# fschmid56/EfficientAT

Hardware: NVIDIA H100
Metric: clips/sec (10s@32kHz) mn10_as fwd+bwd (higher is better)
Workload: dtype f32

## Files before the change

efficientat_b200/engine.py:

```python
import os

import torch

from ._lib import check_module_tensors, lib

ACT = {"none": 0, "relu": 1, "hswish": 2}
BN_EPS = 1e-3
BN_MOM = 0.01


def _ptr(t):
    return 0 if t is None else t.data_ptr()


def _stream():
    return torch.cuda.current_stream().cuda_stream


def _conv_out(n, k, s):
    return (n + 2 * ((k - 1) // 2) - k) // s + 1


class _Layer:
    pass


SE_FUSED_DEFAULT = "1"


DGRAD_BNRED_DEFAULT = "0"


DW_BWD_FUSED_DEFAULT = "1"
DW_BWD_FUSED_SHAPES = ((3, 1), (3, 2), (5, 2))


class _ZeroPool:

    def __init__(self, chunk=1 << 16):
        self.chunk, self.buf, self.off = chunk, None, 0

    def take(self, rows, cols, dev):
        n = rows * cols
        if self.buf is None or self.off + n > self.buf.numel() or self.buf.device != dev:
            self.buf = torch.zeros(max(self.chunk, n), device=dev, dtype=torch.float64)
            self.off = 0
        v = self.buf[self.off:self.off + n].view(rows, cols)
        self.off += n
        return v


class _Fork:

    def __init__(self, device, enabled):
        self.enabled = enabled
        self.side = torch.cuda.Stream(device) if enabled else None
        self.keep = []

    def run(self, fn, *tensors):
        if not self.enabled:
            fn()
            return
        self.side.wait_stream(torch.cuda.current_stream())
        with torch.cuda.stream(self.side):
            fn()
        self.keep.extend(tensors)

    def join(self):
        if self.enabled:
            torch.cuda.current_stream().wait_stream(self.side)
            self.keep.clear()


class MNEngine:
    def __init__(self, model):
        self.model = model
        self.precision = getattr(model, "precision", "fp32")
        if self.precision not in ("fp32", "bf16"):
            raise ValueError(f"precision must be 'fp32' or 'bf16', got {self.precision}")
        self.gemm_impl = os.environ.get("EAT_GEMM", "auto")
        self.tc_min_rows = 1024
        self.pw_impl = "tc" if os.environ.get("EAT_PW_IMPL") == "tc" else "tma"
        self.fork_wgrad = os.environ.get("EAT_FORK_WGRAD", "0") == "1"
        self.se_fused = os.environ.get("EAT_SE_FUSED", SE_FUSED_DEFAULT) == "1"
        self.se_parts_per_sm = int(os.environ.get("EAT_SE_PARTS_PER_SM", "6"))
        self.dgrad_bnred = os.environ.get("EAT_DGRAD_BNRED", DGRAD_BNRED_DEFAULT) == "1"
        self.dw_bwd_fused = os.environ.get("EAT_DW_BWD_FUSED", DW_BWD_FUSED_DEFAULT) == "1"
        self._fork = None
        self._se_scale = {}
        self._zero_pool = _ZeroPool()
        self._plan()

    def _plan(self):
        from .models.mn.block_types import ConcurrentSEBlock, ConvNormActivation, InvertedResidual
        feats = list(self.model.features)
        self.stem = feats[0]
        self.last = feats[-1]
        self.blocks = []
        for m in feats[1:-1]:
            assert isinstance(m, InvertedResidual)
            L = _Layer()
            subs = list(m.block)
            L.expand = L.se = None
            i = 0
            if len([s for s in subs if isinstance(s, ConvNormActivation)]) == 3:
                L.expand = subs[0]
                i = 1
            L.dw = subs[i]
            i += 1
            if isinstance(subs[i], ConcurrentSEBlock):
                L.se = subs[i].conc_se_layers[0]
                i += 1
            L.proj = subs[i]
            L.res = m.use_res_connect
            L.act = ACT["hswish"] if m.cnf.use_hs else ACT["relu"]
            L.k = m.cnf.kernel
            L.stride = m.cnf.stride
            L.cin, L.cexp, L.cout = m.cnf.input_channels, m.cnf.expanded_channels, m.cnf.out_channels
            self.blocks.append(L)
        self.fc1 = self.model.classifier[2]
        self.fc2 = self.model.classifier[5]
        self.dropout_p = self.model.classifier[4].p

    @property
    def tdtype(self):
        return torch.float32 if self.precision == "fp32" else torch.bfloat16

    @property
    def dcode(self):
        return 0 if self.precision == "fp32" else 1

    def _gemm(self, a, w, out, M, N, K, in_sc=None, in_act=0, gate=None, rows_per_sample=1, sc=None, bias=None,
              act=0, res=None, stats=None, a_code=None, c_code=None, w_trans=False):
        a_code = self.dcode if a_code is None else a_code
        c_code = self.dcode if c_code is None else c_code
        scale = _ptr(sc[0]) if sc is not None else 0
        shift = _ptr(sc[1]) if sc is not None else _ptr(bias)
        args = (a.data_ptr(), a_code, w.data_ptr(), 1 if w_trans else 0, out.data_ptr(), c_code, M, N, K,
                _ptr(in_sc[0]) if in_sc is not None else 0, _ptr(in_sc[1]) if in_sc is not None else 0, in_act,
                _ptr(gate), rows_per_sample, scale, shift, act, _ptr(res),
                _ptr(stats[0]) if stats is not None else 0, _ptr(stats[1]) if stats is not None else 0, _stream())
        L = lib()
        use_tc = (self.gemm_impl != "simt" and a_code == c_code and M >= self.tc_min_rows and K % 8 == 0
                  and N % 8 == 0 and act != 3 and in_act != 3)
        if use_tc and a_code == 0 and self.pw_impl == "tma" and not (res is not None and act != 0):
            ws = torch.empty(N * ((K + 31) // 32) * 128, device=w.device, dtype=torch.uint8)
            L.pw_tma_fwd(a.data_ptr(), w.data_ptr(), 1 if w_trans else 0, out.data_ptr(), M, N, K, args[9], args[10], in_act,
                         _ptr(gate), rows_per_sample, scale, shift, act, _ptr(res), args[18], args[19], ws.data_ptr(),
                         ws.numel(), _stream())
        elif use_tc:
            if w_trans:
                wt = torch.empty(N, K, device=w.device, dtype=torch.float32)
                L.transpose_f32(w.data_ptr(), wt.data_ptr(), K, N, _stream())
                args = (args[0], args[1], wt.data_ptr(), 0) + args[4:]
            L.pw_tc_fwd(*args)
        else:
            L.gemm_simt_fwd(*args)

    def _fold(self, bn, dev):
        c = bn.num_features
        sc = torch.empty(2, c, device=dev, dtype=torch.float32)
        lib().bn_fold(bn.weight.data_ptr(), bn.bias.data_ptr(), bn.running_mean.data_ptr(),
                      bn.running_var.data_ptr(), bn.eps, sc[0].data_ptr(), sc[1].data_ptr(), c, _stream())
        return sc

    def _finalize(self, bn, stats, count, dev):
        c = bn.num_features
        sc = torch.empty(2, c, device=dev, dtype=torch.float32)
        sv = torch.empty(2, c, device=dev, dtype=torch.float32)
        mom = bn.momentum if bn.momentum is not None else 0.1
        track = bn.track_running_stats and bn.running_mean is not None
        lib().bn_finalize(stats[0].data_ptr(), stats[1].data_ptr(), float(count), bn.weight.data_ptr(),
                          bn.bias.data_ptr(), bn.eps, mom, _ptr(bn.running_mean) if track else 0,
                          _ptr(bn.running_var) if track else 0, _ptr(bn.num_batches_tracked) if track else 0,
                          sc[0].data_ptr(), sc[1].data_ptr(), sv[0].data_ptr(), sv[1].data_ptr(), c, _stream())
        return sc, sv

    def _se_gate(self, se, pool, inv_count, B, C, dev, hidden=None):
        S = se.fc1.out_features
        key = (S, float(inv_count), str(dev))
        sc = self._se_scale.get(key)
        if sc is None:
            sc = torch.full((S,), float(inv_count), device=dev, dtype=torch.float32)
            self._se_scale[key] = sc
        if hidden is None:
            hidden = torch.empty(B, S, device=dev, dtype=torch.float32)
        self._gemm(pool, se.fc1.weight, hidden, B, S, C, sc=(sc, se.fc1.bias), act=ACT["relu"], a_code=0, c_code=0)
        gate = torch.empty(B, C, device=dev, dtype=torch.float32)
        self._gemm(hidden, se.fc2.weight, gate, B, C, S, bias=se.fc2.bias, act=3, a_code=0, c_code=0)
        return gate, hidden

    def _dw_weights(self, conv, dev):
        c, k = conv.out_channels, conv.kernel_size[0]
        wt = torch.empty(k * k, c, device=dev, dtype=torch.float32)
        lib().dw_repack(conv.weight.data_ptr(), wt.data_ptr(), c, k, _stream())
        return wt

    def forward(self, x, return_fmaps=False):
        if not x.is_cuda:
            raise RuntimeError("efficientat_b200 models run on CUDA (sm_90a) only; got a CPU tensor")
        if x.dim() != 4 or x.shape[1] != 1:
            raise ValueError(f"expected input of shape [B, 1, F, T], got {tuple(x.shape)}")
        check_module_tensors(self.model, x.device, type(self.model).__name__)
        self.dropout_p = float(self.model.classifier[4].p)
        needs_grad = torch.is_grad_enabled() and any(p.requires_grad for p in self.model.parameters())
        with torch.cuda.device(x.device):
            if self.model.training:
                if return_fmaps:
                    raise NotImplementedError("return_fmaps is available in eval mode only")
                from .autograd import mn_train_forward
                logits, feat = mn_train_forward(self, x, needs_grad)
                return self._squeeze(logits, feat) + (None,)
            if needs_grad and x.requires_grad:
                raise NotImplementedError("gradients w.r.t. the input spectrogram are not implemented")
            logits, feat, fmaps = self._forward_eval(x.detach(), return_fmaps)
            return self._squeeze(logits, feat) + (fmaps,)

    @staticmethod
    def _squeeze(logits, feat):
        return logits, feat

    def _forward_eval(self, x, return_fmaps=False):
        L = lib()
        dev = x.device
        st = _stream()
        td, dc = self.tdtype, self.dcode
        x = x.float().contiguous()
        B, _, F, T = x.shape
        fmaps = [] if return_fmaps else None

        def keep(t, f, tt, c):
            if fmaps is not None:
                fmaps.append(t.view(B, f, tt, c).permute(0, 3, 1, 2))

        conv, bn = self.stem[0], self.stem[1]
        s0 = conv.stride[0]
        Fi, Ti = _conv_out(F, 3, s0), _conv_out(T, 3, s0)
        c0 = conv.out_channels
        a = torch.empty(B, Fi, Ti, c0, device=dev, dtype=td)
        sc = self._fold(bn, dev)
# ... 151 lines not shown
                      Fi * Ti, cl, st)
        S["last"] = dict(inp=a, z=zl, sc=scl, sv=svl, Fi=Fi, Ti=Ti)
        n1 = self.fc1.out_features
        h_pre = torch.empty(B, n1, device=dev, dtype=torch.float32)
        self._gemm(feat, self.fc1.weight, h_pre, B, n1, cl, bias=self.fc1.bias, a_code=0, c_code=0)
        p = self.dropout_p
        if dropout_mask is None and p > 0:
            dropout_mask = torch.empty(B, n1, device=dev, dtype=torch.float32).bernoulli_(1.0 - p).div_(1.0 - p)
        ident = self._ident(n1, dev)
        logits = torch.empty(B, self.fc2.out_features, device=dev, dtype=torch.float32)
        self._gemm(h_pre, self.fc2.weight, logits, B, self.fc2.out_features, n1, in_sc=ident, in_act=HS,
                   gate=dropout_mask, rows_per_sample=1, bias=self.fc2.bias, a_code=0, c_code=0)
        S["head"] = dict(feat=feat, h_pre=h_pre, mask=dropout_mask, ident=ident)
        return logits, feat

    def _ident(self, n, dev):
        t = torch.empty(2, n, device=dev, dtype=torch.float32)
        t[0].fill_(1.0)
        t[1].zero_()
        return t

    def _block_modules(self):
        return list(self.model.features)[1:-1]

    def param_list(self):
        return [p for p in self.model.parameters()]

    def _wgrad(self, g, a, dW, db, M, N, K, in_sc=None, in_act=0, gate=None, rows_per_sample=1, g_code=None,
               a_code=None):
        g_code = self.dcode if g_code is None else g_code
        a_code = self.dcode if a_code is None else a_code
        args = (g.data_ptr(), g_code, a.data_ptr(), a_code, dW.data_ptr(), _ptr(db), M, N, K,
                _ptr(in_sc[0]) if in_sc is not None else 0, _ptr(in_sc[1]) if in_sc is not None else 0,
                in_act, _ptr(gate), rows_per_sample, _stream())
        use_tc = (self.gemm_impl != "simt" and db is None and g_code == a_code and M >= self.tc_min_rows
                  and K % 8 == 0 and N % 8 == 0)
        if use_tc:
            lib().pw_tc_wgrad(*args)
        else:
            lib().gemm_simt_wgrad(*args)

    def _bn_bwd_coef(self, gA, gate, dpool, z, sc, sv, act, B, P, C, dgamma, dbeta, dev, code, sums):
        L = lib()
        st = _stream()
        if sums is None:
            s = self._zero_pool.take(2, C, dev)
            L.bn_bwd_reduce(_ptr(gA), _ptr(gate), _ptr(dpool), z.data_ptr(), sc[0].data_ptr(), sc[1].data_ptr(),
                            sv[0].data_ptr(), sv[1].data_ptr(), act, code, B, P, C, s[0].data_ptr(), s[1].data_ptr(), st)
        else:
            s = sums
        coef = torch.empty(2, C, device=dev, dtype=torch.float32)
        L.bn_bwd_finalize(s[0].data_ptr(), s[1].data_ptr(), float(B * P), _ptr(dgamma), _ptr(dbeta),
                          coef[0].data_ptr(), coef[1].data_ptr(), C, st)
        return coef

    def _bn_bwd(self, gA, gate, dpool, z, sc, sv, act, B, P, C, dgamma, dbeta, dev, code=None, sums=None):
        L = lib()
        st = _stream()
        code = self.dcode if code is None else code
        coef = self._bn_bwd_coef(gA, gate, dpool, z, sc, sv, act, B, P, C, dgamma, dbeta, dev, code, sums)
        dz = torch.empty_like(z)
        L.bn_bwd_apply(_ptr(gA), _ptr(gate), _ptr(dpool), z.data_ptr(), sc[0].data_ptr(), sc[1].data_ptr(),
                       sv[0].data_ptr(), sv[1].data_ptr(), act, coef[0].data_ptr(), coef[1].data_ptr(), dz.data_ptr(),
                       code, B, P, C, st)
        return dz

    def _block_bwd(self, blk, R, dy, G, B):
        return self._ir_block_bwd(blk, R, dy, G, B)

    def _ir_block_bwd(self, blk, R, dy, G, B):
        L = lib()
        st = _stream()
        dev = dy.device
        td, dc = self.tdtype, self.dcode
        Fi, Ti, Fo, To = R["Fi"], R["Ti"], R["Fo"], R["To"]
        Pi, Po = Fi * Ti, Fo * To
        gate = R.get("gate")
        dz3 = self._bn_bwd(dy, None, None, R["z3"], R["sc3"], R["sv3"], 0, B, Po, blk.cout,
                           G[blk.proj[1].weight], G[blk.proj[1].bias], dev)
        fork = self._fork if self._fork is not None else _Fork(dev, False)
        fork.run(lambda: self._wgrad(dz3, R["z2"], G[blk.proj[0].weight], None, B * Po, blk.cout, blk.cexp, in_sc=R["sc2"],
                                     in_act=blk.act, gate=gate, rows_per_sample=Po), dz3)
        dp = torch.empty_like(R["z2"])
        self._gemm(dz3, blk.proj[0].weight, dp, B * Po, blk.cexp, blk.cout, w_trans=True)
        dpool = None
        if blk.se is not None:
            Sq = blk.se.fc1.out_features
            dgate = torch.zeros(B, blk.cexp, device=dev, dtype=torch.float32)
            if self.se_fused:
                parts = max(1, min(32, (torch.cuda.get_device_properties(dev).multi_processor_count * self.se_parts_per_sm) // B, (Po + 15) // 16))
                part = torch.empty(parts, 4, B, blk.cexp, device=dev, dtype=torch.float32)
                L.se_bn_bwd_reduce(dp.data_ptr(), R["z2"].data_ptr(), R["sc2"][0].data_ptr(), R["sc2"][1].data_ptr(),
                                   R["sv2"][0].data_ptr(), blk.act, dgate.data_ptr(), part.data_ptr(), parts, dc, B, Po,
                                   blk.cexp, st)
            else:
                L.se_bwd_reduce(dp.data_ptr(), R["z2"].data_ptr(), R["sc2"][0].data_ptr(), R["sc2"][1].data_ptr(),
                                blk.act, dgate.data_ptr(), dc, B, Po, blk.cexp, st)
            du2 = torch.empty(B, blk.cexp, device=dev, dtype=torch.float32)
            du1 = torch.empty(B, Sq, device=dev, dtype=torch.float32)
            dpool = torch.empty(B, blk.cexp, device=dev, dtype=torch.float32)
            L.se_fc_bwd(dgate.data_ptr(), gate.data_ptr(), R["hidden"].data_ptr(), blk.se.fc1.weight.data_ptr(),
                        blk.se.fc2.weight.data_ptr(), 1.0 / Po, du2.data_ptr(), du1.data_ptr(), dpool.data_ptr(),
                        B, blk.cexp, Sq, st)
            fork.run(lambda: (self._wgrad(du2, R["hidden"], G[blk.se.fc2.weight], G[blk.se.fc2.bias], B, blk.cexp, Sq, g_code=0, a_code=0),
                              self._wgrad(du1, R["mean"], G[blk.se.fc1.weight], G[blk.se.fc1.bias], B, Sq, blk.cexp, g_code=0, a_code=0)),
                     du2, du1)
        sums2 = None
        if blk.se is not None and self.se_fused:
            sums2 = self._zero_pool.take(2, blk.cexp, dev)
            L.se_bn_bwd_combine(part.data_ptr(), parts, gate.data_ptr(), dpool.data_ptr(), R["sv2"][1].data_ptr(), B,
                                blk.cexp, sums2[0].data_ptr(), sums2[1].data_ptr(), st)
        has_exp = blk.expand is not None
        dw_in = R["z1"] if has_exp else R["inp"]
        sc1 = R["sc1"] if has_exp else None
        if (self.dw_bwd_fused and dc == 0 and (blk.k, blk.stride) in DW_BWD_FUSED_SHAPES
                and blk.cexp % (4 if blk.k == 3 else 2) == 0):
            coef = self._bn_bwd_coef(dp, gate, dpool, R["z2"], R["sc2"], R["sv2"], blk.act, B, Po, blk.cexp,
                                     G[blk.dw[1].weight], G[blk.dw[1].bias], dev, dc, sums2)
            da1 = torch.empty_like(dw_in)
            sums1 = self._zero_pool.take(2, blk.cexp, dev) if has_exp else None
            L.dw_conv_bwd_fused(dp.data_ptr(), _ptr(gate), _ptr(dpool), R["z2"].data_ptr(), R["sc2"][0].data_ptr(),
                                R["sc2"][1].data_ptr(), R["sv2"][0].data_ptr(), R["sv2"][1].data_ptr(), blk.act,
                                coef[0].data_ptr(), coef[1].data_ptr(), R["wt"].data_ptr(), dw_in.data_ptr(),
                                _ptr(sc1[0]) if has_exp else 0, _ptr(sc1[1]) if has_exp else 0, blk.act if has_exp else 0,
                                _ptr(dy) if (blk.res and not has_exp) else 0, da1.data_ptr(),
                                G[blk.dw[0].weight].data_ptr(), _ptr(R["sv1"][0]) if has_exp else 0,
                                _ptr(R["sv1"][1]) if has_exp else 0, _ptr(sums1[0]) if has_exp else 0,
                                _ptr(sums1[1]) if has_exp else 0, dc, B, Fi, Ti, blk.cexp, blk.k, blk.stride, st)
            return self._expand_bwd(blk, R, dy, G, B, da1, sums1)
        dz2 = self._bn_bwd(dp, gate, dpool, R["z2"], R["sc2"], R["sv2"], blk.act, B, Po, blk.cexp,
                           G[blk.dw[1].weight], G[blk.dw[1].bias], dev, sums=sums2)
        fork.run(lambda: L.dw_conv_wgrad(dz2.data_ptr(), dw_in.data_ptr(), _ptr(sc1[0]) if has_exp else 0,
                                         _ptr(sc1[1]) if has_exp else 0, blk.act if has_exp else 0,
                                         G[blk.dw[0].weight].data_ptr(), 0, dc, B, Fi, Ti, blk.cexp, blk.k, blk.stride,
                                         _stream()), dz2)
        da1 = torch.empty_like(dw_in)
        sums1 = None
        if has_exp and self.dgrad_bnred and blk.stride == 2 and dc == 0 and blk.k in (3, 5):
            sums1 = self._zero_pool.take(2, blk.cexp, dev)
            L.dw_conv_dgrad_bnred(dz2.data_ptr(), R["wt"].data_ptr(), 0, da1.data_ptr(), R["z1"].data_ptr(),
                                  R["sc1"][0].data_ptr(), R["sc1"][1].data_ptr(), R["sv1"][0].data_ptr(),
                                  R["sv1"][1].data_ptr(), blk.act, sums1[0].data_ptr(), sums1[1].data_ptr(), dc, B, Fi, Ti,
                                  blk.cexp, blk.k, blk.stride, st)
        else:
            L.dw_conv_dgrad(dz2.data_ptr(), R["wt"].data_ptr(), 0, _ptr(dy) if (blk.res and not has_exp) else 0,
                            da1.data_ptr(), dc, B, Fi, Ti, blk.cexp, blk.k, blk.stride, st)
        return self._expand_bwd(blk, R, dy, G, B, da1, sums1)

    def _expand_bwd(self, blk, R, dy, G, B, da1, sums1):
        if blk.expand is None:
            return da1
        dev = da1.device
        Pi = R["Fi"] * R["Ti"]
        fork = self._fork if self._fork is not None else _Fork(dev, False)
        dz1 = self._bn_bwd(da1, None, None, R["z1"], R["sc1"], R["sv1"], blk.act, B, Pi, blk.cexp,
                           G[blk.expand[1].weight], G[blk.expand[1].bias], dev, sums=sums1)
        fork.run(lambda: self._wgrad(dz1, R["inp"], G[blk.expand[0].weight], None, B * Pi, blk.cexp, blk.cin), dz1)
        dinp = torch.empty_like(R["inp"])
        self._gemm(dz1, blk.expand[0].weight, dinp, B * Pi, blk.cin, blk.cexp, w_trans=True,
                   res=dy if blk.res else None)
        return dinp

    def _backward(self, S, dlogits, on_ready=None):
        L = lib()
        st = _stream()
        dev = dlogits.device
        td, dc = self.tdtype, self.dcode
        B = S["B"]
        HS = ACT["hswish"]
        self._zero_pool = _ZeroPool()
        params = self.param_list()
        flat = torch.zeros(sum(p.numel() for p in params), device=dev, dtype=torch.float32)
        G, off = {}, 0
        for p in params:
            G[p] = flat[off:off + p.numel()].view_as(p)
            off += p.numel()
        dlogits = dlogits.float().contiguous()
        fork = self._fork = _Fork(dev, self.fork_wgrad)
        pidx = {id(p): i for i, p in enumerate(params)}

        def done(module):
            fork.join()
            if on_ready is not None:
                on_ready(flat, min(pidx[id(p)] for p in module.parameters()))

        H = S["head"]
        n1, ncls, cl = self.fc1.out_features, self.fc2.out_features, self.fc1.in_features
        fork.run(lambda: self._wgrad(dlogits, H["h_pre"], G[self.fc2.weight], G[self.fc2.bias], B, ncls, n1, in_sc=H["ident"],
                                     in_act=HS, gate=H["mask"], rows_per_sample=1, g_code=0, a_code=0), dlogits)
        dh = torch.empty(B, n1, device=dev, dtype=torch.float32)
        self._gemm(dlogits, self.fc2.weight, dh, B, n1, ncls, a_code=0, c_code=0, w_trans=True)
        dpre = torch.empty_like(dh)
        L.act_bwd(dh.data_ptr(), H["h_pre"].data_ptr(), _ptr(H["mask"]), HS, dpre.data_ptr(), dh.numel(), st)
        fork.run(lambda: self._wgrad(dpre, H["feat"], G[self.fc1.weight], G[self.fc1.bias], B, n1, cl, g_code=0, a_code=0), dpre)
        dfeat = torch.empty(B, cl, device=dev, dtype=torch.float32)
        self._gemm(dpre, self.fc1.weight, dfeat, B, cl, n1, a_code=0, c_code=0, w_trans=True)
        done(self.fc1)

        Ls = S["last"]
        P = Ls["Fi"] * Ls["Ti"]
        conv, bn = self.last[0], self.last[1]
        dpool = dfeat.mul_(1.0 / P)
        dz = self._bn_bwd(None, None, dpool, Ls["z"], Ls["sc"], Ls["sv"], HS, B, P, cl, G[bn.weight], G[bn.bias], dev)
        fork.run(lambda: self._wgrad(dz, Ls["inp"], G[conv.weight], None, B * P, cl, conv.in_channels), dz)
        dy = torch.empty_like(Ls["inp"])
        self._gemm(dz, conv.weight, dy, B * P, conv.in_channels, cl, w_trans=True)
        done(self.last)

        for blk, R, mod in zip(reversed(self.blocks), reversed(S["blocks"]), reversed(self._block_modules())):
            dy = self._block_bwd(blk, R, dy, G, B)
            done(mod)
        St = S["stem"]
        conv, bn = self.stem[0], self.stem[1]
        c0 = conv.out_channels
        dz0 = self._bn_bwd(dy, None, None, St["z"], St["sc"], St["sv"], HS, B, St["Fo"] * St["To"], c0, G[bn.weight],
                           G[bn.bias], dev)
        L.stem_wgrad(dz0.data_ptr(), dc, S["x"].data_ptr(), G[conv.weight].data_ptr(), B, S["F"], S["T"], c0,
                     conv.stride[0], st)
        fork.join()
        self._fork = None
        G[None] = flat
        return G
```

include/eat_b200.h:

```cpp
#ifndef EAT_B200_H
#define EAT_B200_H

#ifndef __CUDA_RUNTIME_H__
typedef struct CUstream_st* cudaStream_t;
#endif

#ifdef __cplusplus
extern "C" {
#endif

#define EAT_OK 0
#define EAT_ERR_ARG 1
#define EAT_ERR_CUDA 2
#define EAT_ERR_UNSUPPORTED 3

#define EAT_ACT_NONE 0
#define EAT_ACT_RELU 1
#define EAT_ACT_HSWISH 2
#define EAT_ACT_SIGMOID 3

#define EAT_F32 0
#define EAT_BF16 1

const char* eat_last_error(void);
int eat_abi_version(void);

int eat_dw_plan(int kind, int dtype, int B, int F, int T, int C, int k, int stride, int per_sample, int* plan);
int eat_device_check(int device);

int eat_mel_fwd(const float* wave, int B, int N, const float* window, int win_length, int hop, int n_fft,
                const float* twiddle, const int* fb_start, const int* fb_len, const float* fb_w, int max_len,
                int n_mels, float preemph, float* out, cudaStream_t stream);

int eat_mel_filterbank(int n_mels, int n_fft, float sample_rate, double fmin, double fmax, int* fb_start,
                       int* fb_len, float* fb_w, int cap, cudaStream_t stream);

int eat_mel_mask(float* spec, int B, int F, int T, const int* f_start, const int* f_end, const int* t_start,
                 const int* t_end, float fill, cudaStream_t stream);

int eat_stem_fwd(const float* x, const float* w, void* out, int out_dtype, int B, int F, int T, int C, int stride,
                 const float* scale, const float* shift, int act, double* stat_sum, double* stat_sq,
                 cudaStream_t stream);

int eat_dw_repack(const float* w, float* wt, int C, int k, cudaStream_t stream);

int eat_dw_conv_fwd(const void* in, const float* wt, void* out, int dtype, int B, int F, int T, int C, int k,
                    int stride, const float* in_scale, const float* in_shift, int in_act, const float* scale,
                    const float* shift, int act, float* pool, double* stat_sum, double* stat_sq,
                    cudaStream_t stream);

int eat_bn_fold(const float* gamma, const float* beta, const float* rmean, const float* rvar, float eps,
                float* scale, float* shift, int C, cudaStream_t stream);

int eat_bn_finalize(const double* sum, const double* sq, double count, const float* gamma, const float* beta,
                    float eps, float momentum, float* rmean, float* rvar, long long* nbt, float* scale,
                    float* shift, float* save_mean, float* save_invstd, int C, cudaStream_t stream);

int eat_bn_apply(const void* z, const float* scale, const float* shift, int act, const void* res, void* y,
                 int dtype, long long rows, int C, cudaStream_t stream);

int eat_bn_act_pool(const void* z, const float* scale, const float* shift, int act, float* pool, float mul,
                    int dtype, int B, int P, int C, cudaStream_t stream);

int eat_se_fc_fwd(const float* pool, float inv_count, const float* w1, const float* b1, const float* w2,
                  const float* b2, float* gate, float* hidden_out, int B, int C, int S, cudaStream_t stream);

int eat_gemm_simt_fwd(const void* A, int a_dtype, const float* W, int w_trans, void* C, int c_dtype, long long M,
                      int N, int K, const float* in_scale, const float* in_shift, int in_act, const float* gate,
                      int rows_per_sample, const float* scale, const float* shift, int act, const void* residual,
                      double* stat_sum, double* stat_sq, cudaStream_t stream);

int eat_pw_tc_fwd(const void* A, int a_dtype, const float* W, int w_trans, void* C, int c_dtype, long long M, int N,
                  int K, const float* in_scale, const float* in_shift, int in_act, const float* gate,
                  int rows_per_sample, const float* scale, const float* shift, int act, const void* residual,
                  double* stat_sum, double* stat_sq, cudaStream_t stream);
int eat_pw_tma_fwd(const float* A, const float* W, int w_trans, float* C, long long M, int N, int K,
                   const float* in_scale, const float* in_shift, int in_act, const float* gate, int rows_per_sample,
                   const float* scale, const float* shift, int act, const float* residual, double* stat_sum,
                   double* stat_sq, void* w_ws, long long w_ws_bytes, cudaStream_t stream);
int eat_pw_tma_dyn_fwd(const float* A, const float* W, const float* att, int dyn_k, int w_trans, float* C, long long M,
                       int N, int K, int rows_per_sample, const float* scale, const float* shift, int act,
                       const float* residual, double* stat_sum, double* stat_sq, void* w_ws, long long w_ws_bytes,
                       cudaStream_t stream);
int eat_transpose_f32(const float* in, float* out, int rows, int cols, cudaStream_t stream);


int eat_pw_tc_dyn_fwd(const void* A, int dtype, const float* W, const float* att, int dyn_k, void* C, long long M,
                      int N, int K, int rows_per_sample, const float* in_scale, const float* in_shift, int in_act,
                      const float* scale, const float* shift, int act, const void* residual, double* stat_sum,
                      double* stat_sq, cudaStream_t stream);
int eat_dw_conv_fwd_dy(const void* in, const float* wt, long long wt_bstride, void* out, int dtype, int B, int F, int T,
                       int C, int k, int stride, const float* in_scale, const float* in_shift, int in_act,
                       const float* scale, const float* shift, const float* theta, const float* lam,
                       const float* init, const float* ca_f, const float* ca_t, double* stat_sum, double* stat_sq,
                       cudaStream_t stream);
int eat_ctx_pool(const void* x, int dtype, float* out, int B, int F, int T, int C, cudaStream_t stream);
int eat_seq_pool(const float* in, float* out, int B, int Ltot, int row0, int L, int H, int stride, const float* scale,
                 const float* shift, int act, cudaStream_t stream);
int eat_dyconv_att(const float* hc, const float* wr, const float* br, float temperature, float* att, int B, int H, int k,
                   cudaStream_t stream);
int eat_dyconv_mix_dw(const float* w, const float* att, float* wt, int B, int C, int ksize, int k, cudaStream_t stream);

int eat_dy_act_fwd(const void* z, void* out, int dtype, const float* scale, const float* shift, const float* theta,
                   const float* lam, const float* init, const float* ca_f, const float* ca_t, int B, int Fo, int To,
                   int C, cudaStream_t stream);
int eat_dy_act_bwd(const void* dp, const void* z, void* du, int dtype, const float* scale, const float* shift,
                   const float* theta, const float* lam, const float* init, const float* ca_f, const float* ca_t,
                   float* dcaf, float* dcat, float* dcoef, int B, int Fo, int To, int C, cudaStream_t stream);
int eat_dyrelu_coef_bwd(const float* dcoef, const float* theta, const float* lam, float* dpre, long long n,
                        cudaStream_t stream);
int eat_sigmoid_bwd(const float* g, const float* s, float* out, long long n, cudaStream_t stream);
int eat_dyconv_att_bwd(const float* datt, const float* att, float temperature, const float* hc, const float* wr,
                       float* dwr, float* dbr, float* dhc, int B, int H, int k, cudaStream_t stream);
int eat_seq_pool_bwd(const float* dout, float* dsrc, int B, int Ltot, int row0, int L, int H, int stride,
                     cudaStream_t stream);
int eat_ctx_pool_bwd(const float* dg, void* dx, int dtype, int B, int F, int T, int C, cudaStream_t stream);
int eat_pw_tc_wgrad_persample(const void* G, const void* A, int dtype, float* S, long long M, int N, int K,
                              int rows_per_sample, cudaStream_t stream);
int eat_dyn_wgrad_mix(const float* S, const float* att, const float* W, float* dW, float* datt, int B, long long n, int k,
                      cudaStream_t stream);


int eat_gemm_simt_wgrad(const void* G, int g_dtype, const void* A, int a_dtype, float* dW, float* db, long long M,
                        int N, int K, const float* in_scale, const float* in_shift, int in_act, const float* gate,
                        int rows_per_sample, cudaStream_t stream);

int eat_pw_tc_wgrad(const void* G, int g_dtype, const void* A, int a_dtype, float* dW, float* db, long long M, int N,
                    int K, const float* in_scale, const float* in_shift, int in_act, const float* gate,
                    int rows_per_sample, cudaStream_t stream);

int eat_pw_tma_wgrad(const float* G, const float* X, float* dW, long long M, int N, int K, const float* in_scale,
                     const float* in_shift, int in_act, const float* gate, int rows_per_sample, int per_sample,
                     cudaStream_t stream);

int eat_bn_bwd_reduce(const void* gA, const float* gate, const float* dpool, const void* z, const float* scale,
                      const float* shift, const float* mean, const float* invstd, int act, int dtype, int B, int P,
                      int C, double* s1, double* s2, cudaStream_t stream);
int eat_bn_bwd_finalize(const double* s1, const double* s2, double count, float* dgamma, float* dbeta, float* c1,
                        float* c2, int C, cudaStream_t stream);
int eat_bn_bwd_apply(const void* gA, const float* gate, const float* dpool, const void* z, const float* scale,
                     const float* shift, const float* mean, const float* invstd, int act, const float* c1,
                     const float* c2, void* dz, int dtype, int B, int P, int C, cudaStream_t stream);

int eat_se_bwd_reduce(const void* dp, const void* z, const float* scale, const float* shift, int act, float* dgate,
                      int dtype, int B, int P, int C, cudaStream_t stream);
int eat_se_bn_bwd_reduce(const void* dp, const void* z, const float* scale, const float* shift, const float* mean, int act,
                         float* dgate, float* part, int parts, int dtype, int B, int P, int C, cudaStream_t stream);
int eat_se_bn_bwd_combine(const float* part, int parts, const float* gate, const float* dpool, const float* invstd, int B,
                          int C, double* s1, double* s2, cudaStream_t stream);
int eat_se_fc_bwd(const float* dgate, const float* gate, const float* hidden, const float* w1, const float* w2,
                  float inv_count, float* du2, float* du1, float* dpool, int B, int C, int S, cudaStream_t stream);

int eat_dw_conv_dgrad(const void* dz, const float* wt, long long wt_bstride, const void* res, void* din, int dtype, int B,
                      int F, int T, int C, int k, int stride, cudaStream_t stream);
int eat_dw_conv_dgrad_s1(const void* dz, const float* wt, long long wt_bstride, const void* res, void* din, int dtype,
                         int B, int F, int T, int C, int k, cudaStream_t stream);
int eat_dw_conv_dgrad_bnred(const void* dz, const float* wt, const void* res, void* din, const void* z, const float* zscale,
                            const float* zshift, const float* zmean, const float* zinvstd, int zact, double* s1, double* s2,
                            int dtype, int B, int F, int T, int C, int k, int stride, cudaStream_t stream);
int eat_dw_conv_wgrad(const void* dz, const void* in, const float* in_scale, const float* in_shift, int in_act,
                      float* dw, long long dw_bstride, int dtype, int B, int F, int T, int C, int k, int stride,
                      cudaStream_t stream);
int eat_dw_conv_bwd_fused(const float* dp, const float* gate, const float* dpool, const float* z2, const float* scale,
                          const float* shift, const float* mean, const float* invstd, int act, const float* c1,
                          const float* c2, const float* wt, const float* in, const float* in_scale, const float* in_shift,
                          int in_act, const float* res, float* din, float* dw, const float* zmean, const float* zinvstd,
                          double* s1, double* s2, int dtype, int B, int F, int T, int C, int k, int stride,
                          cudaStream_t stream);
int eat_stem_wgrad(const void* dz, int dtype, const float* x, float* dw, int B, int F, int T, int C, int stride,
                   cudaStream_t stream);
int eat_act_bwd(const float* dh, const float* pre, const float* mask, int act, float* dpre, long long n,
                cudaStream_t stream);


int eat_mixup(const float* x, const int* perm, const float* lam, float* out, int B, long long per_sample,
              cudaStream_t stream);
int eat_bce_kd_loss(const float* logits, const float* y, const float* teacher, const float* teacher_known,
                    const int* perm, const float* lam, float kd_lambda, int B, int C, float* dlogits,
                    double* loss_acc, cudaStream_t stream);
int eat_adam_step(float* p, const float* g, float* m, float* v, long long n, float lr, float beta1, float beta2,
                  float eps, float weight_decay, int adamw, int step, float grad_scale, cudaStream_t stream);

#ifdef __cplusplus
}
#endif
#endif
```

Before: 4666.

## Fuse expand pointwise backward: BN/act bwd, dgrad and wgrad in one TMA/WGMMA kernel

Adds a warp-specialized kernel that applies the BN and activation backward to the expand-conv output gradient on the fly in shared memory, then computes both the input gradient (plus residual) and the weight gradient with WGMMA in a single pass. The engine routes expand-block backward through it when cexp<=128 and cin<=32 in fp32. This avoids materializing dz1 and reading it twice through separate GEMM launches. In exchange the weight gradient is reduced with atomics, which makes it nondeterministic, and the kernel uses split hi/lo operands with a deep TMA pipeline.

```diff
diff --git a/efficientat_b200/csrc/pw_bwd_fused.cu b/efficientat_b200/csrc/pw_bwd_fused.cu
--- /dev/null
+++ b/efficientat_b200/csrc/pw_bwd_fused.cu
@@ -0,0 +1,364 @@
+#include "tma_common.cuh"
+
+namespace {
+using namespace tc;
+using namespace tma;
+
+constexpr int BM = 128;
+constexpr int BOX = BM * 128;
+constexpr int kThreads = 416;
+constexpr int kFirstCons = 4, kTmaWarp = 12;
+constexpr int STG_BYTES = 16 * 128;
+constexpr int kMaxKb = 4;
+constexpr int kMaxStages = 6;
+constexpr size_t kSmemLimit = 227 * 1024;
+
+struct PbParams {
+  const float *scale, *shift, *mean, *invstd, *c1, *c2, *W;
+  float* dW;
+  int M, cexp, cin, m_tiles, stages, res;
+  uint32_t off_x, off_w, off_stg, off_f, off_bar;
+};
+
+struct PbPlan { int splits, rows_per_split, stages, smem, nkb; uint32_t off_x, off_w, off_stg, off_f, off_bar; };
+
+int plan_pb(long long M, int cexp, int cin, int sms, PbPlan& pl) {
+  if (M < 1 || cexp < 1 || cin < 1) { eat_set_error("pw_conv_bwd_fused: M, cexp and cin must be positive"); return EAT_ERR_ARG; }
+  if (cexp % 4 != 0 || cin % 4 != 0) { eat_set_error("pw_conv_bwd_fused: cexp and cin must be multiples of 4 (16-byte row pitch for TMA)"); return EAT_ERR_ARG; }
+  if (M >= (1ll << 31) - BM) { eat_set_error("pw_conv_bwd_fused: M too large"); return EAT_ERR_ARG; }
+  if (cin > KB || cexp > kMaxKb * KB) {
+    eat_set_error("pw_conv_bwd_fused: cin <= 32 and cexp <= 128 only (register-resident weight gradient)");
+    return EAT_ERR_UNSUPPORTED;
+  }
+  pl.nkb = (cexp + KB - 1) / KB;
+  const int m_tiles = (int)((M + BM - 1) / BM);
+  pl.splits = m_tiles < sms ? m_tiles : sms;
+  pl.rows_per_split = ((m_tiles + pl.splits - 1) / pl.splits) * BM;
+  const size_t x_bytes = 2 * 2 * (size_t)BOX, w_bytes = (size_t)pl.nkb * KB * 128, stg = 8 * 2 * (size_t)STG_BYTES;
+  const size_t floats = 4 * (size_t)pl.nkb * KB * 4, bars = (3 * (size_t)kMaxStages + 6) * 8;
+  const size_t fixed = x_bytes + w_bytes + stg + floats + bars + 1024 ;
+  pl.stages = (int)((kSmemLimit - fixed) / (2 * BOX));
+  if (pl.stages > kMaxStages) pl.stages = kMaxStages;
+  if (pl.stages < 2) { eat_set_error("pw_conv_bwd_fused: shared-memory budget exceeded"); return EAT_ERR_UNSUPPORTED; }
+  size_t off = (size_t)pl.stages * 2 * BOX;
+  pl.off_x = (uint32_t)off; off += x_bytes;
+  pl.off_w = (uint32_t)off; off += w_bytes;
+  pl.off_stg = (uint32_t)off; off += stg;
+  pl.off_f = (uint32_t)off; off += floats;
+  pl.off_bar = (uint32_t)off; off += (3 * (size_t)pl.stages + 6) * 8;
+  pl.smem = (int)off;
+  return EAT_OK;
+}
+
+template <int ACT>
+__device__ __forceinline__ void fix_dz(unsigned char* dat, const unsigned char* zt, int ft, int rows_valid, const float* s_sc,
+                                       const float* s_sh, const float* s_al, const float* s_be, int k) {
+  const int cp = ft & 3, r0 = ft >> 2;
+  const uint32_t row_off = (uint32_t)((r0 >> 3) * 1024 + (r0 & 7) * 128);
+  const int x = r0 & 7;
+  const uint32_t in0 = row_off + (((2 * cp) ^ x) << 4), in1 = row_off + (((2 * cp + 1) ^ x) << 4);
+  const uint32_t out_hi = row_off + ((cp ^ x) << 4), out_lo = row_off + (((4 + cp) ^ x) << 4);
+  float sc[8], sh[8], al[8], be[8];
+#pragma unroll
+  for (int j = 0; j < 8; ++j) { sc[j] = s_sc[k + j]; sh[j] = s_sh[k + j]; al[j] = s_al[k + j]; be[j] = s_be[k + j]; }
+#pragma unroll
+  for (int i = 0; i < 4; ++i) {
+    const uint32_t o = (uint32_t)i * 32 * 128;
+    const float4 ga = *reinterpret_cast<const float4*>(dat + in0 + o), gb = *reinterpret_cast<const float4*>(dat + in1 + o);
+    const float4 za = *reinterpret_cast<const float4*>(zt + in0 + o), zb = *reinterpret_cast<const float4*>(zt + in1 + o);
+    const float g[8] = {ga.x, ga.y, ga.z, ga.w, gb.x, gb.y, gb.z, gb.w};
+    const float zv[8] = {za.x, za.y, za.z, za.w, zb.x, zb.y, zb.z, zb.w};
+    float d[8];
+    const bool live = r0 + 32 * i < rows_valid;
+#pragma unroll
+    for (int j = 0; j < 8; ++j) {
+      const float gg = g[j] * act_bwd(fmaf(zv[j], sc[j], sh[j]), ACT);
+      d[j] = live ? fmaf(sc[j], gg, fmaf(al[j], zv[j], be[j])) : 0.f;
+    }
+    __syncwarp();
+    uint4 h, l;
+    split8(make_float4(d[0], d[1], d[2], d[3]), make_float4(d[4], d[5], d[6], d[7]), h, l);
+    *reinterpret_cast<uint4*>(dat + out_hi + o) = h;
+    *reinterpret_cast<uint4*>(dat + out_lo + o) = l;
+  }
+}
+
+template <int NKB, int ACT>
+__global__ void __launch_bounds__(kThreads, 1)
+pw_bwd_fused_kernel(const __grid_constant__ CUtensorMap mapDA, const __grid_constant__ CUtensorMap mapZ,
+                    const __grid_constant__ CUtensorMap mapX, const __grid_constant__ CUtensorMap mapR,
+                    const __grid_constant__ CUtensorMap mapC, const PbParams p) {
+  constexpr int KP = NKB * KB;
+  constexpr int NWA = (NKB + 1) / 2;
+  extern __shared__ __align__(1024) unsigned char smem[];
+  unsigned char* s_x = smem + p.off_x;
+  unsigned char* s_w = smem + p.off_w;
+  unsigned char* s_stg = smem + p.off_stg;
+  float* s_sc = reinterpret_cast<float*>(smem + p.off_f);
+  float* s_sh = s_sc + KP;
+  float* s_al = s_sh + KP;
+  float* s_be = s_al + KP;
+  uint64_t* bars = reinterpret_cast<uint64_t*>(smem + p.off_bar);
+  const int S = p.stages;
+  const uint32_t bar_full = smem_u32(bars), bar_ready = bar_full + 8 * S, bar_empty = bar_ready + 8 * S;
+  const uint32_t bar_tfull = bar_empty + 8 * S, bar_tready = bar_tfull + 16, bar_tempty = bar_tready + 16;
+
+  const int warp = threadIdx.x >> 5, lane = threadIdx.x & 31;
+  const int t_begin = (int)((long long)blockIdx.x * p.m_tiles / gridDim.x);
+  const int t_end = (int)((long long)(blockIdx.x + 1) * p.m_tiles / gridDim.x);
+  if (threadIdx.x == 0) {
+    for (int s = 0; s < S; ++s) { mbar_init(bar_full + 8 * s, 1); mbar_init(bar_ready + 8 * s, 4); mbar_init(bar_empty + 8 * s, 2); }
+    for (int s = 0; s < 2; ++s) { mbar_init(bar_tfull + 8 * s, 1); mbar_init(bar_tready + 8 * s, 4); mbar_init(bar_tempty + 8 * s, 2); }
+    asm volatile("fence.mbarrier_init.release.cluster;" ::: "memory");
+    asm volatile("prefetch.tensormap [%0];" ::"l"(reinterpret_cast<uint64_t>(&mapDA)) : "memory");
+    asm volatile("prefetch.tensormap [%0];" ::"l"(reinterpret_cast<uint64_t>(&mapZ)) : "memory");
+    asm volatile("prefetch.tensormap [%0];" ::"l"(reinterpret_cast<uint64_t>(&mapX)) : "memory");
+    asm volatile("prefetch.tensormap [%0];" ::"l"(reinterpret_cast<uint64_t>(&mapC)) : "memory");
+  }
+  for (int c = threadIdx.x; c < KP; c += kThreads) {
+    float sc = 0.f, sh = 0.f, al = 0.f, be = 0.f;
+    if (c < p.cexp) {
+      sc = p.scale[c]; sh = p.shift[c];
+      al = -sc * p.c2[c] * p.invstd[c];
+      be = -sc * p.c1[c] - al * p.mean[c];
+    }
+    s_sc[c] = sc; s_sh[c] = sh; s_al[c] = al; s_be[c] = be;
+  }
+  for (int i = threadIdx.x; i < NKB * KB * 4; i += kThreads) {
+    const int cp = i & 3, n = (i >> 2) & (KB - 1), kb = i >> 7;
+    float v[8];
+#pragma unroll
+    for (int j = 0; j < 8; ++j) {
+      const int k = kb * KB + cp * 8 + j;
+      v[j] = (n < p.cin && k < p.cexp) ? __ldg(p.W + (size_t)k * p.cin + n) : 0.f;
+    }
+    uint4 hi, lo;
+    split8(make_float4(v[0], v[1], v[2], v[3]), make_float4(v[4], v[5], v[6], v[7]), hi, lo);
+    unsigned char* wt = s_w + (size_t)kb * KB * 128;
+    *reinterpret_cast<uint4*>(wt + swz(n, cp)) = hi;
+    *reinterpret_cast<uint4*>(wt + swz(n, 4 + cp)) = lo;
+  }
+  fence_proxy_async();
+  __syncthreads();
+  const uint32_t stage_base = smem_u32(smem), x_base = smem_u32(s_x);
+
+  if (warp == kTmaWarp) {
+    if (lane == 0) {
+      int s = 0;
+      uint32_t ph = 0;
+      for (int t = t_begin, i = 0; t < t_end; ++t, ++i) {
+        const int slot = i & 1;
+        const uint32_t tph = (uint32_t)(i >> 1) & 1u;
+        const int m0 = t * BM;
+        mbar_wait(bar_tempty + 8 * slot, tph ^ 1u);
+        const uint32_t xd = x_base + (uint32_t)slot * 2 * BOX;
+        mbar_expect_tx(bar_tfull + 8 * slot, (uint32_t)(p.res ? 2 : 1) * BOX);
+        tma_load_2d(&mapX, bar_tfull + 8 * slot, xd, 0, m0);
+        if (p.res) tma_load_2d(&mapR, bar_tfull + 8 * slot, xd + BOX, 0, m0);
+        for (int kb = 0; kb < NKB; ++kb) {
+          mbar_wait(bar_empty + 8 * s, ph ^ 1u);
+          const uint32_t dst = stage_base + (uint32_t)s * 2 * BOX;
+          mbar_expect_tx(bar_full + 8 * s, 2 * BOX);
+          tma_load_2d(&mapDA, bar_full + 8 * s, dst, kb * KB, m0);
+          tma_load_2d(&mapZ, bar_full + 8 * s, dst + BOX, kb * KB, m0);
+          if (++s == S) { s = 0; ph ^= 1u; }
+        }
+      }
+    }
+    __syncwarp();
+  } else if (warp < kFirstCons) {
+    const int ft = threadIdx.x;
+    int s = 0;
+    uint32_t ph = 0;
+    for (int t = t_begin, i = 0; t < t_end; ++t, ++i) {
+      const int slot = i & 1;
+      const uint32_t tph = (uint32_t)(i >> 1) & 1u;
+      const int rows_valid = min(BM, p.M - t * BM);
+      mbar_wait(bar_tfull + 8 * slot, tph);
+      fix_a<2, -1>(s_x + (size_t)slot * 2 * BOX, ft, rows_valid, nullptr, nullptr, 0, nullptr, 0, 0, 1, 0);
+      fence_proxy_async();
+      __syncwarp();
+      if (lane == 0) mbar_arrive(bar_tready + 8 * slot);
+      for (int kb = 0; kb < NKB; ++kb) {
+        mbar_wait(bar_full + 8 * s, ph);
+        unsigned char* st = smem + (size_t)s * 2 * BOX;
+        fix_dz<ACT>(st, st + BOX, ft, rows_valid, s_sc, s_sh, s_al, s_be, kb * KB + (ft & 3) * 8);
+        fence_proxy_async();
+        __syncwarp();
+        if (lane == 0) mbar_arrive(bar_ready + 8 * s);
+        if (++s == S) { s = 0; ph ^= 1u; }
+      }
+    }
+  } else {
+    const int cw = warp - kFirstCons;
+    const int g = cw >> 2, wq = cw & 3;
+    const int ctid = threadIdx.x - kFirstCons * 32;
+    unsigned char* stg = s_stg + (size_t)cw * 2 * STG_BYTES;
+    const uint64_t desc0 = gmma_desc(0);
+    const uint64_t w0 = desc0 + (smem_u32(s_w) >> 4);
+    const int fr = lane >> 2, fc = 2 * (lane & 3);
+    float accW[NWA][32];
+#pragma unroll
+    for (int w = 0; w < NWA; ++w)
+#pragma unroll
+      for (int e = 0; e < 32; ++e) accW[w][e] = 0.f;
+    int s = 0, cb = 0;
+    uint32_t ph = 0;
+    for (int t = t_begin, i = 0; t < t_end; ++t, ++i) {
+      const int slot = i & 1;
+      const uint32_t tph = (uint32_t)(i >> 1) & 1u;
+      mbar_wait(bar_tready + 8 * slot, tph);
+      if (p.res) mbar_wait(bar_tfull + 8 * slot, tph);
+      const uint32_t sx = x_base + (uint32_t)slot * 2 * BOX;
+      float acc[16];
+#pragma unroll
+      for (int e = 0; e < 16; ++e) acc[e] = 0.f;
+#pragma unroll
+      for (int kb = 0; kb < NKB; ++kb) {
+        mbar_wait(bar_ready + 8 * s, ph);
+        const uint32_t sa = stage_base + (uint32_t)s * 2 * BOX;
+        const uint64_t a_hi = desc0 + ((sa + (uint32_t)g * 8192u) >> 4), a_lo = a_hi + 4;
+        const uint64_t w_hi = w0 + (uint64_t)(kb * KB * 128 / 16), w_lo = w_hi + 4;
+        wgmma_fence();
+#pragma unroll
+        for (int j = 0; j < 2; ++j) {
+          const uint64_t ko = (uint64_t)(j * 2);
+          wgmma_n32<0, 0>(acc, a_hi + ko, w_hi + ko);
+          wgmma_n32<0, 0>(acc, a_lo + ko, w_hi + ko);
+          wgmma_n32<0, 0>(acc, a_hi + ko, w_lo + ko);
+        }
+        if ((kb & 1) == g) {
+#pragma unroll
+          for (int st = 0; st < BM / 16; ++st)
+            wgmma_n64<1, 1>(accW[kb >> 1], gmma_desc(sa + st * 2048, BOX, 1024), gmma_desc(sx + st * 2048, BOX, 1024));
+        }
+        wgmma_commit();
+        wgmma_wait<0>();
+        wgmma_fence_regs(acc);
+#pragma unroll
+        for (int w = 0; w < NWA; ++w) wgmma_fence_regs(accW[w]);
+        asm volatile("bar.sync %0, 128;" ::"r"(1 + g) : "memory");
+        if (ctid == g * 128) mbar_arrive(bar_empty + 8 * s);
+        if (++s == S) { s = 0; ph ^= 1u; }
+      }
+      const int rl = g * 64 + wq * 16;
+      const int row0 = t * BM + rl;
+      unsigned char* buf = stg + (size_t)cb * STG_BYTES;
+      cb ^= 1;
+      if (lane == 0) tma_wait_read<1>();
+      __syncwarp();
+      const unsigned char* rt = s_x + (size_t)slot * 2 * BOX + BOX;
+#pragma unroll
+      for (int j = 0; j < 4; ++j) {
+        const int cc = 8 * j + fc;
+        float2 v0 = make_float2(acc[4 * j], acc[4 * j + 1]), v1 = make_float2(acc[4 * j + 2], acc[4 * j + 3]);
+        if (p.res) {
+          const float2 r0 = *reinterpret_cast<const float2*>(rt + swz(rl + fr, cc >> 2) + (cc & 3) * 4);
+          const float2 r1 = *reinterpret_cast<const float2*>(rt + swz(rl + fr + 8, cc >> 2) + (cc & 3) * 4);
+          v0.x += r0.x; v0.y += r0.y; v1.x += r1.x; v1.y += r1.y;
+        }
+        const uint32_t co = (uint32_t)(((cc >> 2) << 4) + (cc & 3) * 4);
+        *reinterpret_cast<float2*>(buf + fr * 128 + (co ^ ((fr & 7) << 4))) = v0;
+        *reinterpret_cast<float2*>(buf + (fr + 8) * 128 + (co ^ (((fr + 8) & 7) << 4))) = v1;
+      }
+      fence_proxy_async();
+      __syncwarp();
+      if (lane == 0 && row0 < p.M) { tma_store_2d(&mapC, smem_u32(buf), 0, row0); tma_commit(); }
+      asm volatile("bar.sync %0, 128;" ::"r"(1 + g) : "memory");
+      if (ctid == g * 128) mbar_arrive(bar_tempty + 8 * slot);
+    }
+    if (t_end > t_begin) {
+      const bool hi_row = wq < 2;
+#pragma unroll
+      for (int w = 0; w < NWA; ++w) {
+        const int kb = 2 * w + g;
+        if (kb >= NKB) continue;
+#pragma unroll
+        for (int h = 0; h < 2; ++h) {
+          const int n = kb * KB + (wq & 1) * 16 + (lane >> 2) + 8 * h;
+          if (n >= p.cexp) continue;
+#pragma unroll
+          for (int j = 0; j < 4; ++j) {
+            const int k = 8 * j + 2 * (lane & 3);
+            float2 v = make_float2(accW[w][4 * j + 2 * h], accW[w][4 * j + 2 * h + 1]);
+            if (hi_row) { v.x += accW[w][4 * (j + 4) + 2 * h]; v.y += accW[w][4 * (j + 4) + 2 * h + 1]; }
+            if (k < p.cin) atomicAdd(reinterpret_cast<float2*>(p.dW + (size_t)n * p.cin + k), v);
+          }
+        }
+      }
+    }
+    if (lane == 0) tma_wait_read<0>();
+    __syncwarp();
+  }
+  __syncthreads();
+}
+
+template <int NKB, int ACT>
+int launch_pb(const CUtensorMap& mDA, const CUtensorMap& mZ, const CUtensorMap& mX, const CUtensorMap& mR,
+              const CUtensorMap& mC, const PbParams& p, const PbPlan& pl, cudaStream_t st) {
+  static unsigned long long attr_mask = 0;
+  if (int rc = eat_opt_in_smem(pw_bwd_fused_kernel<NKB, ACT>, kSmemLimit, attr_mask)) return rc;
+  pw_bwd_fused_kernel<NKB, ACT><<<pl.splits, kThreads, pl.smem, st>>>(mDA, mZ, mX, mR, mC, p);
+  EAT_CHECK_LAUNCH();
+  return EAT_OK;
+}
+
+template <int ACT>
+int launch_pb_act(const CUtensorMap& mDA, const CUtensorMap& mZ, const CUtensorMap& mX, const CUtensorMap& mR,
+                  const CUtensorMap& mC, const PbParams& p, const PbPlan& pl, cudaStream_t st) {
+  switch (pl.nkb) {
+    case 1: return launch_pb<1, ACT>(mDA, mZ, mX, mR, mC, p, pl, st);
+    case 2: return launch_pb<2, ACT>(mDA, mZ, mX, mR, mC, p, pl, st);
+    case 3: return launch_pb<3, ACT>(mDA, mZ, mX, mR, mC, p, pl, st);
+    default: return launch_pb<4, ACT>(mDA, mZ, mX, mR, mC, p, pl, st);
+  }
+}
+
+}
+
+extern "C" int eat_pw_bwd_plan(long long M, int cexp, int cin, int* plan) {
+  if (plan == nullptr) { eat_set_error("pw_bwd_plan: plan is NULL"); return EAT_ERR_ARG; }
+  PbPlan pl;
+  if (int rc = plan_pb(M, cexp, cin, kNumSMs, pl)) return rc;
+  plan[0] = pl.splits; plan[1] = pl.rows_per_split; plan[2] = pl.stages; plan[3] = pl.smem;
+  return EAT_OK;
+}
+
+extern "C" int eat_pw_conv_bwd_fused(const float* da, const float* z, const float* scale, const float* shift,
+                                     const float* mean, const float* invstd, int act, const float* c1, const float* c2,
+                                     const float* X, const float* W, const float* res, float* dX, float* dW, int dtype,
+                                     long long M, int cexp, int cin, cudaStream_t st) {
+  if (dtype != EAT_F32) { eat_set_error("pw_conv_bwd_fused: fp32 storage only"); return EAT_ERR_UNSUPPORTED; }
+  if (act != EAT_ACT_RELU && act != EAT_ACT_HSWISH) { eat_set_error("pw_conv_bwd_fused: activation must be relu or hardswish"); return EAT_ERR_UNSUPPORTED; }
+  if (M < 0) { eat_set_error("pw_conv_bwd_fused: negative M"); return EAT_ERR_ARG; }
+  if (da == nullptr || z == nullptr || scale == nullptr || shift == nullptr || mean == nullptr || invstd == nullptr ||
+      c1 == nullptr || c2 == nullptr || X == nullptr || W == nullptr || dX == nullptr || dW == nullptr) {
+    eat_set_error("pw_conv_bwd_fused: da, z, the BatchNorm tables, c1/c2, X, W, dX and dW are required");
+    return EAT_ERR_ARG;
+  }
+  if ((((uintptr_t)da) | ((uintptr_t)z) | ((uintptr_t)X) | ((uintptr_t)res) | ((uintptr_t)dX)) & 15) {
+    eat_set_error("pw_conv_bwd_fused: activation tensors must be 16-byte aligned");
+    return EAT_ERR_ARG;
+  }
+  if (((uintptr_t)dW) & 7) { eat_set_error("pw_conv_bwd_fused: dW must be 8-byte aligned"); return EAT_ERR_ARG; }
+  PbPlan pl;
+  if (int rc = plan_pb(M > 0 ? M : 1, cexp, cin, kNumSMs, pl)) return rc;
+  if (M == 0) return EAT_OK;
+  int dev = 0, sms = kNumSMs;
+  cudaGetDevice(&dev);
+  cudaDeviceGetAttribute(&sms, cudaDevAttrMultiProcessorCount, dev);
+  if (int rc = plan_pb(M, cexp, cin, sms, pl)) return rc;
+  CUtensorMap mDA, mZ, mX, mR, mC;
+  if (int rc = make_map(&mDA, da, M, cexp, BM)) return rc;
+  if (int rc = make_map(&mZ, z, M, cexp, BM)) return rc;
+  if (int rc = make_map(&mX, X, M, cin, BM)) return rc;
+  if (int rc = make_map(&mR, res != nullptr ? res : X, M, cin, BM)) return rc;
+  if (int rc = make_map(&mC, dX, M, cin, 16)) return rc;
+  PbParams p;
+  p.scale = scale; p.shift = shift; p.mean = mean; p.invstd = invstd; p.c1 = c1; p.c2 = c2; p.W = W; p.dW = dW;
+  p.M = (int)M; p.cexp = cexp; p.cin = cin; p.m_tiles = (int)((M + BM - 1) / BM); p.stages = pl.stages;
+  p.res = res != nullptr ? 1 : 0;
+  p.off_x = pl.off_x; p.off_w = pl.off_w; p.off_stg = pl.off_stg; p.off_f = pl.off_f; p.off_bar = pl.off_bar;
+  if (act == EAT_ACT_RELU) return launch_pb_act<EAT_ACT_RELU>(mDA, mZ, mX, mR, mC, p, pl, st);
+  return launch_pb_act<EAT_ACT_HSWISH>(mDA, mZ, mX, mR, mC, p, pl, st);
+}
diff --git a/efficientat_b200/engine.py b/efficientat_b200/engine.py
--- a/efficientat_b200/engine.py
+++ b/efficientat_b200/engine.py
@@ -33,6 +33,9 @@
 
 DW_BWD_FUSED_DEFAULT = "1"
 DW_BWD_FUSED_SHAPES = ((3, 1), (3, 2), (5, 2))
+
+
+EXPAND_BWD_FUSED_DEFAULT = "1"
 
 
 class _ZeroPool:
@@ -86,6 +89,8 @@
         self.se_parts_per_sm = int(os.environ.get("EAT_SE_PARTS_PER_SM", "6"))
         self.dgrad_bnred = os.environ.get("EAT_DGRAD_BNRED", DGRAD_BNRED_DEFAULT) == "1"
         self.dw_bwd_fused = os.environ.get("EAT_DW_BWD_FUSED", DW_BWD_FUSED_DEFAULT) == "1"
+        self.expand_bwd_fused = os.environ.get("EAT_EXPAND_BWD_FUSED", EXPAND_BWD_FUSED_DEFAULT) == "1"
+        self._pw_bwd_ok = {}
         self._fork = None
         self._se_scale = {}
         self._zero_pool = _ZeroPool()
@@ -543,6 +548,17 @@
             return da1
         dev = da1.device
         Pi = R["Fi"] * R["Ti"]
+        if self.expand_bwd_fused and self.dcode == 0 and self._pw_bwd_fused_takes(B * Pi, blk.cexp, blk.cin):
+            coef = self._bn_bwd_coef(da1, None, None, R["z1"], R["sc1"], R["sv1"], blk.act, B, Pi, blk.cexp,
+                                     G[blk.expand[1].weight], G[blk.expand[1].bias], dev, 0, sums1)
+            dinp = torch.empty_like(R["inp"])
+            sc1, sv1 = R["sc1"], R["sv1"]
+            lib().pw_conv_bwd_fused(da1.data_ptr(), R["z1"].data_ptr(), sc1[0].data_ptr(), sc1[1].data_ptr(),
+                                    sv1[0].data_ptr(), sv1[1].data_ptr(), blk.act, coef[0].data_ptr(), coef[1].data_ptr(),
+                                    R["inp"].data_ptr(), blk.expand[0].weight.data_ptr(), _ptr(dy) if blk.res else 0,
+                                    dinp.data_ptr(), G[blk.expand[0].weight].data_ptr(), 0, B * Pi, blk.cexp, blk.cin,
+                                    _stream())
+            return dinp
         fork = self._fork if self._fork is not None else _Fork(dev, False)
         dz1 = self._bn_bwd(da1, None, None, R["z1"], R["sc1"], R["sv1"], blk.act, B, Pi, blk.cexp,
                            G[blk.expand[1].weight], G[blk.expand[1].bias], dev, sums=sums1)
@@ -551,6 +567,19 @@
         self._gemm(dz1, blk.expand[0].weight, dinp, B * Pi, blk.cin, blk.cexp, w_trans=True,
                    res=dy if blk.res else None)
         return dinp
+
+    def _pw_bwd_fused_takes(self, M, cexp, cin):
+        key = (M, cexp, cin)
+        if key not in self._pw_bwd_ok:
+            import ctypes
+            from ._lib import EatError
+            plan = (ctypes.c_int * 4)()
+            try:
+                lib().pw_bwd_plan(M, cexp, cin, ctypes.addressof(plan))
+                self._pw_bwd_ok[key] = True
+            except EatError:
+                self._pw_bwd_ok[key] = False
+        return self._pw_bwd_ok[key]
 
     def _backward(self, S, dlogits, on_ready=None):
         L = lib()
diff --git a/include/eat_b200.h b/include/eat_b200.h
--- a/include/eat_b200.h
+++ b/include/eat_b200.h
@@ -167,6 +167,11 @@
                           int in_act, const float* res, float* din, float* dw, const float* zmean, const float* zinvstd,
                           double* s1, double* s2, int dtype, int B, int F, int T, int C, int k, int stride,
                           cudaStream_t stream);
+int eat_pw_conv_bwd_fused(const float* da, const float* z, const float* scale, const float* shift, const float* mean,
+                          const float* invstd, int act, const float* c1, const float* c2, const float* X, const float* W,
+                          const float* res, float* dX, float* dW, int dtype, long long M, int cexp, int cin,
+                          cudaStream_t stream);
+int eat_pw_bwd_plan(long long M, int cexp, int cin, int* plan);
 int eat_stem_wgrad(const void* dz, int dtype, const float* x, float* dw, int B, int F, int T, int C, int stride,
                    cudaStream_t stream);
 int eat_act_bwd(const float* dh, const float* pre, const float* mask, int act, float* dpre, long long n,
```

New measurement: 4984, median of 6. +6.8%, better.
